# ds2-lab/LambdaFS

Measured on AMD Instinct MI355X. Metric: RS encode+decode GiB/s device-resident; 1/2/4/8 MI355X; %HBM roofline, higher is better.
Workload: dtype u8; 1 GPU; RS(10,4) encode + 1-erasure decode (data shard 0), 1024 KiB cells, 1024 stripes/GPU, device-resident; encodeBulk / decodeBulk via hrs_encode_dev / hrs_decode_dev; stripes_per_gpu=1024, stripes_total=1024, cell_bytes=1048576, k=10, p=4, parallelism=stripe-sharded x1 (RCCL: matrix broadcast + barriers only)

## Files before the change

lambdafs_amd/csrc/hrs_device.hpp:

```cpp
#pragma once
#include <hip/hip_runtime.h>

#include <cstdint>
#include <type_traits>

#include "gf256.hpp"
#include "hrs_crc.hpp"
#include "hrs_internal.hpp"
#include "xor_sched.hpp"

namespace hrs {

typedef uint32_t u32x4 __attribute__((ext_vector_type(4)));

__device__ __forceinline__ uint32_t xor3(uint32_t a, uint32_t b, uint32_t c) {
  return __builtin_amdgcn_bitop3_b32(a, b, c, 0x96);
}

__device__ __forceinline__ uint32_t bsel(uint32_t m, uint32_t x, uint32_t y) {
  return __builtin_amdgcn_bitop3_b32(m, x, y, 0xCA);
}

template <int SH, uint32_t M>
__device__ __forceinline__ void xchg(uint32_t& a, uint32_t& b) {
  const uint32_t na = bsel(M << SH, b << SH, a);
  const uint32_t nb = bsel(M, a >> SH, b);
  a = na;
  b = nb;
}

__device__ __forceinline__ void bitslice(uint32_t (&w)[8]) {
  xchg<1, 0x55555555u>(w[0], w[1]);
  xchg<1, 0x55555555u>(w[2], w[3]);
  xchg<1, 0x55555555u>(w[4], w[5]);
  xchg<1, 0x55555555u>(w[6], w[7]);
  xchg<2, 0x33333333u>(w[0], w[2]);
  xchg<2, 0x33333333u>(w[1], w[3]);
  xchg<2, 0x33333333u>(w[4], w[6]);
  xchg<2, 0x33333333u>(w[5], w[7]);
  xchg<4, 0x0F0F0F0Fu>(w[0], w[4]);
  xchg<4, 0x0F0F0F0Fu>(w[1], w[5]);
  xchg<4, 0x0F0F0F0Fu>(w[2], w[6]);
  xchg<4, 0x0F0F0F0Fu>(w[3], w[7]);
}

__device__ __forceinline__ void xtime(uint32_t (&p)[8]) {
  const uint32_t hi = p[7];
  p[7] = p[6];
  p[6] = p[5];
  p[5] = p[4];
  p[4] = p[3] ^ hi;
  p[3] = p[2] ^ hi;
  p[2] = p[1] ^ hi;
  p[1] = p[0];
  p[0] = hi;
}

__device__ __forceinline__ void load_row(const uint8_t* p, int lane, uint32_t (&w)[8]) {
  const u32x4 x = __builtin_nontemporal_load(reinterpret_cast<const u32x4*>(p + lane * 16));
  const u32x4 y = __builtin_nontemporal_load(reinterpret_cast<const u32x4*>(p + 1024 + lane * 16));
  w[0] = x[0]; w[1] = x[1]; w[2] = x[2]; w[3] = x[3];
  w[4] = y[0]; w[5] = y[1]; w[6] = y[2]; w[7] = y[3];
}

__device__ __forceinline__ void store_row(uint8_t* p, int lane, const uint32_t (&w)[8]) {
  const u32x4 x = {w[0], w[1], w[2], w[3]};
  const u32x4 y = {w[4], w[5], w[6], w[7]};
  __builtin_nontemporal_store(x, reinterpret_cast<u32x4*>(p + lane * 16));
  __builtin_nontemporal_store(y, reinterpret_cast<u32x4*>(p + 1024 + lane * 16));
}

typedef __attribute__((address_space(1))) u32x4 g_u32x4;

__device__ __forceinline__ uint64_t uniform_addr(const void* p) {
  const uint64_t v = reinterpret_cast<uint64_t>(p);
  const uint32_t lo = __builtin_amdgcn_readfirstlane(static_cast<uint32_t>(v));
  const uint32_t hi = __builtin_amdgcn_readfirstlane(static_cast<uint32_t>(v >> 32));
  return (static_cast<uint64_t>(hi) << 32) | lo;
}

__device__ __forceinline__ void load_row_u(const uint8_t* base, uint32_t loff, uint32_t (&w)[8]) {
  const g_u32x4* b = reinterpret_cast<const g_u32x4*>(uniform_addr(base) + loff);
  const u32x4 x = __builtin_nontemporal_load(b);
  const u32x4 y = __builtin_nontemporal_load(b + 64);
  w[0] = x[0]; w[1] = x[1]; w[2] = x[2]; w[3] = x[3];
  w[4] = y[0]; w[5] = y[1]; w[6] = y[2]; w[7] = y[3];
}

__device__ __forceinline__ void store_row_u(uint8_t* base, uint32_t loff, const uint32_t (&w)[8]) {
  g_u32x4* b = reinterpret_cast<g_u32x4*>(uniform_addr(base) + loff);
  const u32x4 x = {w[0], w[1], w[2], w[3]};
  const u32x4 y = {w[4], w[5], w[6], w[7]};
  __builtin_nontemporal_store(x, b);
  __builtin_nontemporal_store(y, b + 64);
}

__device__ __forceinline__ uint32_t wave_id_in_grid() {
  return __builtin_amdgcn_readfirstlane(blockIdx.x * (blockDim.x >> 6) + (threadIdx.x >> 6));
}

struct WaveTasks {
  uint64_t t0, end, jump;
  uint32_t chunk, wpb;

  __device__ __forceinline__ uint64_t at(uint32_t j) const {
    if (chunk == 1) return t0 + j * jump;
    const uint32_t q = j / chunk;
    return t0 + q * jump + static_cast<uint64_t>(j - q * chunk) * wpb;
  }
};

__device__ __forceinline__ WaveTasks wave_tasks(uint64_t ntasks, int order) {
  const uint32_t wpb = blockDim.x >> 6;
  const uint32_t w = __builtin_amdgcn_readfirstlane(threadIdx.x >> 6);
  if (order >= 1) {
    const uint32_t c = static_cast<uint32_t>(order);
    return {static_cast<uint64_t>(blockIdx.x) * c * wpb + w, ntasks, static_cast<uint64_t>(gridDim.x) * c * wpb, c, wpb};
  }
  const uint64_t per = (ntasks + gridDim.x - 1) / gridDim.x;
  const uint64_t lo = per * blockIdx.x;
  return {lo + w, lo + per < ntasks ? lo + per : ntasks, 0, 0xFFFFFFFFu, wpb};
}

template <int K, int P, class MATRIX>
struct StaticPlan {
  uint8_t mask[P][K][8];
  constexpr StaticPlan() : mask{} {
    const MATRIX g;
    for (int o = 0; o < P; ++o)
      for (int r = 0; r < K; ++r)
        for (int q = 0; q < 8; ++q) mask[o][r][q] = gf::row_mask(g.m[o][r], q);
  }
};

template <int K, int P, class MATRIX>
__device__ __forceinline__ void encode_row_acc(int r, const uint32_t (&w)[8], uint32_t (&acc)[P][8],
                                               uint32_t (&pend)[P][8], bool (&has)[P][8]) {
  constexpr StaticPlan<K, P, MATRIX> plan{};
#pragma unroll
  for (int o = 0; o < P; ++o)
#pragma unroll
    for (int q = 0; q < 8; ++q) {
#pragma unroll
      for (int i = 0; i < 8; ++i) {
        if ((plan.mask[o][r][q] >> i) & 1) {
          if (has[o][q]) {
            acc[o][q] = xor3(acc[o][q], pend[o][q], w[i]);
            has[o][q] = false;
          } else {
            pend[o][q] = w[i];
            has[o][q] = true;
          }
        }
      }
    }
}


template <int B, int E, class F>
__device__ __forceinline__ void static_for(F&& f) {
  if constexpr (B < E) {
    f(std::integral_constant<int, B>{});
    static_for<B + 1, E>(f);
  }
}

template <class MATRIX> struct MatrixFamily;
template <int K, int P> struct MatrixFamily<gf::EncodeMatrix<K, P>> { static constexpr int value = 0; };
template <int K, int P> struct MatrixFamily<gf::CauchyMatrix<K, P>> { static constexpr int value = 1; };

template <class S, int GI, int G, int P>
__device__ __forceinline__ void xor_sched_apply(const uint32_t (&x)[G][8], uint32_t (&acc)[P][8]) {
  constexpr int nin = S::kNin[GI];
  constexpr int op0 = S::kOpOff[GI];
  constexpr int nops = S::kOpOff[GI + 1] - op0;
  uint32_t v[S::kMaxVars];
#pragma unroll
  for (int i = 0; i < nin; ++i) v[i] = x[i >> 3][i & 7];
  static_for<0, nops>([&](auto j) __attribute__((always_inline)) {
    constexpr xsched::Op op = S::kOps[op0 + decltype(j)::value];
    if constexpr (op.c == 255)
      v[nin + decltype(j)::value] = v[op.a] ^ v[op.b];
    else
      v[nin + decltype(j)::value] = xor3(v[op.a], v[op.b], v[op.c]);
  });
  static_for<0, 8 * P>([&](auto pl) __attribute__((always_inline)) {
    constexpr int t0 = S::kTermOff[GI][decltype(pl)::value];
    constexpr int t1 = S::kTermOff[GI][decltype(pl)::value + 1];
    uint32_t& a = acc[decltype(pl)::value >> 3][decltype(pl)::value & 7];
    int t = t0;
    if constexpr (GI == 0) {
      if constexpr (t1 == t0) {
        a = 0u;
      } else {
        a = v[S::kTerms[t0]];
        t = t0 + 1;
      }
    }
#pragma unroll
    for (; t + 1 < t1; t += 2) a = xor3(a, v[S::kTerms[t]], v[S::kTerms[t + 1]]);
    if (t < t1) a ^= v[S::kTerms[t]];
  });
}


__device__ __forceinline__ uint32_t zmul(const uint32_t* z, uint32_t c) {
  return z[c & 0xFFu] ^ z[256 + ((c >> 8) & 0xFFu)] ^ z[512 + ((c >> 16) & 0xFFu)] ^ z[768 + (c >> 24)];
}

typedef __attribute__((address_space(3))) const uint32_t lds_u32;

struct SliceTab {
  uint32_t lw_lo;
  uint32_t lw_hi;
};

__device__ __forceinline__ SliceTab slice_tab(int lane, uint32_t rep_mask = kCrcRep - 1) {
  const uint32_t c4 = (static_cast<uint32_t>(lane) & rep_mask) * 4u;
  return SliceTab{c4, c4 | 0x10000u};
}

__device__ __forceinline__ uint32_t lds_at(uint32_t byte_addr) {
  return *reinterpret_cast<lds_u32*>(static_cast<uintptr_t>(byte_addr));
}

__device__ __forceinline__ uint32_t slice4(const SliceTab& t, uint32_t x) {
  const uint32_t a3 = __builtin_amdgcn_perm(x, t.lw_hi, 0x0C020400u);
  const uint32_t a2 = __builtin_amdgcn_perm(x, t.lw_hi, 0x0C020500u);
  const uint32_t a1 = __builtin_amdgcn_perm(x, t.lw_lo, 0x0C0C0600u);
  const uint32_t a0 = __builtin_amdgcn_perm(x, t.lw_lo, 0x0C0C0700u);
  return xor3(lds_at(a3 + 128u), lds_at(a2), lds_at(a1 + 128u)) ^ lds_at(a0);
}

__device__ __forceinline__ uint32_t slice4_xor(const SliceTab& t, uint32_t x, uint32_t y) {
  const uint32_t a3 = __builtin_amdgcn_perm(x, t.lw_hi, 0x0C020400u);
  const uint32_t a2 = __builtin_amdgcn_perm(x, t.lw_hi, 0x0C020500u);
  const uint32_t a1 = __builtin_amdgcn_perm(x, t.lw_lo, 0x0C0C0600u);
  const uint32_t a0 = __builtin_amdgcn_perm(x, t.lw_lo, 0x0C0C0700u);
  return xor3(xor3(lds_at(a3 + 128u), lds_at(a2), lds_at(a1 + 128u)), lds_at(a0), y);
}

__device__ __forceinline__ uint32_t piece_crc(const SliceTab& s, uint32_t w0, uint32_t w1, uint32_t w2, uint32_t w3) {
  uint32_t c = slice4_xor(s, w0, w1);
  c = slice4_xor(s, c, w2);
  c = slice4_xor(s, c, w3);
  return slice4(s, c);
}

__device__ __forceinline__ uint32_t zmul_xor(const uint32_t* z, uint32_t c, uint32_t y) {
  return xor3(xor3(z[c & 0xFFu], z[256 + ((c >> 8) & 0xFFu)], z[512 + ((c >> 16) & 0xFFu)]), z[768 + (c >> 24)], y);
}

template <int M>
__device__ __forceinline__ void rows_piece_crcs(const SliceTab& t, const uint32_t (&x)[M][8], uint32_t (&c0)[M],
                                                uint32_t (&c1)[M]) {
#pragma unroll
  for (int m = 0; m < M; ++m) {
    c0[m] = x[m][0];
    c1[m] = x[m][4];
  }
#pragma unroll
  for (int st = 0; st < 4; ++st) {
#pragma unroll
    for (int m = 0; m < M; ++m) {
      c0[m] = slice4(t, c0[m]);
      c1[m] = slice4(t, c1[m]);
    }
    if (st < 3) {
#pragma unroll
      for (int m = 0; m < M; ++m) {
        c0[m] ^= x[m][st + 1];
        c1[m] ^= x[m][st + 5];
      }
    }
// ... 127 lines not shown
```

lambdafs_amd/csrc/hrs_internal.hpp:

```cpp
#pragma once
#include <cstddef>
#include <cstdint>
#include <hip/hip_runtime.h>

namespace hrs {

constexpr int kMaxIn = 32;
constexpr int kMaxInRuntime = 16;
constexpr int kMaxInRuntimeWide = 8;
inline int runtime_in_chunk(int nout) { return nout <= 5 ? kMaxInRuntime : kMaxInRuntimeWide; }
constexpr int kMaxOut = 8;

constexpr int kWindowBytes = 2048;
constexpr int kBlockThreads = 256;
constexpr int kWavesPerBlock = kBlockThreads / 64;

struct RowArgs {
  const uint8_t* in[kMaxIn];
  uint8_t* out[kMaxOut];
  uint64_t cw[kMaxIn];
  uint64_t in_stride;
  uint64_t out_stride;
  uint64_t len;
  uint64_t nwin;
  uint64_t ntasks;
  int nin;
  int nout;
  int accumulate;
  int order;
};

inline void set_coef(RowArgs& a, int o, int i, uint8_t v) {
  a.cw[i] = (a.cw[i] & ~(0xFFull << (8 * o))) | (static_cast<uint64_t>(v) << (8 * o));
}

enum class KernelKind : int {
  kStaticEncode = 0,
  kBitsliced = 1,
  kBytewise = 2,
};

enum { kStaticRs = 0, kStaticCauchy = 1 };
hipError_t launch_static_encode(int family, int k, int p, const RowArgs& a, hipStream_t s, bool* handled);
hipError_t launch_bitsliced(const RowArgs& a, hipStream_t s);
hipError_t launch_bitsliced_stream(const RowArgs& a, hipStream_t s);
hipError_t launch_bytewise(const RowArgs& a, hipStream_t s);
hipError_t launch_xor(const RowArgs& a, hipStream_t s);
int device_cu_count();

void note_kernel(const char* name);
const char* last_kernel();


constexpr int kBatchMaxIn = 32;
constexpr int kHostBatchSlots = 3;
constexpr int kAsyncSlots = 4;
constexpr int kHostSlots = 8;
struct BatchPlan {
  int nin;
  int nout;
  int loc[kBatchMaxIn];
  uint64_t cw[kBatchMaxIn];
};

struct BatchArgs {
  const uint8_t* base;
  uint8_t* out;
  uint64_t row_stride, stripe_stride, out_row_stride, out_stripe_stride;
  uint64_t len;
  uint64_t col0;
  uint64_t nwin;
  uint64_t ntasks;
  const BatchPlan* plans;
  const int32_t* pat;
  int order;
  int pad_;
};

hipError_t launch_batch_bitsliced(const BatchArgs& a, int max_nout, int max_nin, hipStream_t s);


constexpr int kScrubHead = 4;
constexpr int kScrubPatched = 3;
constexpr uint32_t kScrubNone = 0xFFFFFFFFu;
constexpr int kScrubMaxRows = 255;

struct ScrubArgs {
  const uint8_t* rows[kScrubMaxRows];
  uint64_t stride;
  uint64_t len;
  uint64_t col0;
  uint64_t nwin;
  uint64_t ntasks;
  uint32_t* reports;
  uint64_t report_stride;
  int n, p;
  int order;
  int pad_;
};

hipError_t launch_scrub_init(uint32_t* reports, uint64_t report_stride, int n, uint64_t nstripes, hipStream_t s);
hipError_t launch_scrub(const ScrubArgs& a, hipStream_t s);
hipError_t launch_scrub_bytewise(const ScrubArgs& a, hipStream_t s);
hipError_t launch_heal(const ScrubArgs& a, hipStream_t s);
hipError_t launch_heal_bytewise(const ScrubArgs& a, hipStream_t s);

hipError_t launch_batch_bytewise(const BatchArgs& a, hipStream_t s);

}
```

lambdafs_amd/csrc/hrs_kernels.hip:

```cpp
#include <hip/hip_runtime.h>

#include <cstdlib>
#include <string>

#include "hrs_device.hpp"
#include "hrs_launch.hpp"

namespace hrs {
namespace {


__constant__ gf::Tables d_tables = gf::make_tables();


template <int K, int P, class MATRIX>
__device__ __forceinline__ void encode_static_body(const RowArgs& a) {
  const int lane = threadIdx.x & 63;
  const WaveTasks wt = wave_tasks(a.ntasks, a.order);
  for (uint32_t j = 0; j < 0xFFFFFFFFu; ++j) {
    const uint64_t t = wt.at(j);
    if (t >= wt.end) break;
    const uint64_t stripe = t / a.nwin;
    const uint64_t off = (t - stripe * a.nwin) * kWindowBytes;
    uint32_t acc[P][8];
    uint32_t pend[P][8];
    bool has[P][8];
#pragma unroll
    for (int o = 0; o < P; ++o)
#pragma unroll
      for (int q = 0; q < 8; ++q) {
        acc[o][q] = 0u;
        pend[o][q] = 0u;
        has[o][q] = false;
      }
#pragma unroll
    for (int r = 0; r < K; ++r) {
      uint32_t w[8];
      load_row(a.in[r] + stripe * a.in_stride + off, lane, w);
      bitslice(w);
      encode_row_acc<K, P, MATRIX>(r, w, acc, pend, has);
    }
#pragma unroll
    for (int o = 0; o < P; ++o)
#pragma unroll
      for (int q = 0; q < 8; ++q)
        if (has[o][q]) acc[o][q] ^= pend[o][q];
#pragma unroll
    for (int o = 0; o < P; ++o) {
      bitslice(acc[o]);
      store_row(a.out[o] + stripe * a.out_stride + off, lane, acc[o]);
    }
  }
}

template <int K, int P>
__global__ void __launch_bounds__(kBlockThreads) encode_static_kernel(const RowArgs a) {
  encode_static_body<K, P, gf::EncodeMatrix<K, P>>(a);
}

template <int K, int P>
__global__ void __launch_bounds__(kBlockThreads) encode_cauchy_kernel(const RowArgs a) {
  encode_static_body<K, P, gf::CauchyMatrix<K, P>>(a);
}


template <int NINB>
__global__ void __launch_bounds__(kBlockThreads) xor_kernel(const RowArgs a) {
  const int lane = threadIdx.x & 63;
  const int nin = a.nin;
  const WaveTasks wt = wave_tasks(a.ntasks, a.order);
  for (uint32_t j = 0; j < 0xFFFFFFFFu; ++j) {
    const uint64_t t = wt.at(j);
    if (t >= wt.end) break;
    const uint64_t stripe = t / a.nwin;
    const uint64_t off = (t - stripe * a.nwin) * kWindowBytes;
    const uint64_t in_base = stripe * a.in_stride + off;
    uint32_t rows[NINB][8];
#pragma unroll
    for (int r = 0; r < NINB; ++r)
      if (r < nin) load_row(a.in[r] + in_base, lane, rows[r]);
    uint32_t acc[8];
    if (a.accumulate) {
      load_row(a.out[0] + stripe * a.out_stride + off, lane, acc);
    } else {
#pragma unroll
      for (int q = 0; q < 8; ++q) acc[q] = 0u;
    }
#pragma unroll
    for (int r = 0; r < NINB; r += 2) {
      if (r + 1 < nin) {
#pragma unroll
        for (int q = 0; q < 8; ++q) acc[q] = xor3(acc[q], rows[r][q], rows[r + 1][q]);
      } else if (r < nin) {
#pragma unroll
        for (int q = 0; q < 8; ++q) acc[q] ^= rows[r][q];
      }
    }
    store_row(a.out[0] + stripe * a.out_stride + off, lane, acc);
  }
}


__global__ void __launch_bounds__(kBlockThreads) bytewise_kernel(const RowArgs a) {
  __shared__ uint8_t s_exp[512];
  __shared__ uint8_t s_log[256];
  for (int i = threadIdx.x; i < 512; i += blockDim.x) s_exp[i] = d_tables.exp[i];
  for (int i = threadIdx.x; i < 256; i += blockDim.x) s_log[i] = d_tables.log[i];
  __syncthreads();
  const uint64_t nthreads = static_cast<uint64_t>(gridDim.x) * blockDim.x;
  for (uint64_t idx = static_cast<uint64_t>(blockIdx.x) * blockDim.x + threadIdx.x; idx < a.ntasks;
       idx += nthreads) {
    const uint64_t stripe = idx / a.len;
    const uint64_t col = idx - stripe * a.len;
    uint8_t acc[kMaxOut];
#pragma unroll
    for (int o = 0; o < kMaxOut; ++o)
      acc[o] = (a.accumulate && o < a.nout) ? a.out[o][stripe * a.out_stride + col] : 0;
    for (int r = 0; r < a.nin; ++r) {
      const uint8_t x = a.in[r][stripe * a.in_stride + col];
      if (x == 0) continue;
      const int lx = s_log[x];
#pragma unroll
      for (int o = 0; o < kMaxOut; ++o) {
        const uint8_t c = static_cast<uint8_t>(a.cw[r] >> (8 * o));
        if (o < a.nout && c != 0) acc[o] ^= s_exp[lx + s_log[c]];
      }
    }
#pragma unroll
    for (int o = 0; o < kMaxOut; ++o)
      if (o < a.nout) a.out[o][stripe * a.out_stride + col] = acc[o];
  }
}

template <int K, int P>
hipError_t launch_static(const RowArgs& a, hipStream_t s) {
  auto kern = encode_static_kernel<K, P>;
  note_kernel_t("encode_static_kernel", K, P);
  const unsigned g = stream_grid(a.ntasks);
  hipLaunchKernelGGL(kern, dim3(g), dim3(kBlockThreads), 0, s, with_order(a, kOrderStaticEncode));
  return hipGetLastError();
}

template <int K, int P>
hipError_t launch_cauchy(const RowArgs& a, hipStream_t s) {
  auto kern = encode_cauchy_kernel<K, P>;
  note_kernel_t("encode_cauchy_kernel", K, P);
  const unsigned g = stream_grid(a.ntasks);
  hipLaunchKernelGGL(kern, dim3(g), dim3(kBlockThreads), 0, s, with_order(a, kOrderStaticEncode));
  return hipGetLastError();
}

}

int device_cu_count() { return device_cus(); }

namespace {
thread_local std::string t_last_kernel;
}
void note_kernel(const char* name) { t_last_kernel = name; }
const char* last_kernel() { return t_last_kernel.c_str(); }

hipError_t launch_static_encode(int family, int k, int p, const RowArgs& a, hipStream_t s, bool* handled) {
  *handled = true;
  if (family == kStaticCauchy) {
    if (k == 10 && p == 4) return launch_cauchy<10, 4>(a, s);
    if (k == 6 && p == 3) return launch_cauchy<6, 3>(a, s);
    *handled = false;
    return hipSuccess;
  }
  if (k == 10 && p == 4) return launch_static<10, 4>(a, s);
  if (k == 6 && p == 3) return launch_static<6, 3>(a, s);
  if (k == 3 && p == 2) return launch_static<3, 2>(a, s);
  if (k == 12 && p == 4) return launch_static<12, 4>(a, s);
  *handled = false;
  return hipSuccess;
}

template <int NINB>
hipError_t launch_xor_n(const RowArgs& a, hipStream_t s) {
  auto kern = xor_kernel<NINB>;
  note_kernel_t("xor_kernel", NINB);
  hipLaunchKernelGGL(kern, dim3(stream_grid(a.ntasks)), dim3(kBlockThreads), 0, s, with_order(a, kOrderStaticEncode));
  return hipGetLastError();
}

hipError_t launch_xor(const RowArgs& a, hipStream_t s) {
  if (a.nin <= 4) return launch_xor_n<4>(a, s);
  if (a.nin <= 8) return launch_xor_n<8>(a, s);
  if (a.nin <= 12) return launch_xor_n<12>(a, s);
  if (a.nin <= 16) return launch_xor_n<16>(a, s);
  return hipErrorInvalidValue;
}

hipError_t launch_bytewise(const RowArgs& a, hipStream_t s) {
  const unsigned g = grid_for(bytewise_kernel, kBlockThreads, a.ntasks);
  note_kernel("bytewise_kernel");
  hipLaunchKernelGGL(bytewise_kernel, dim3(g), dim3(kBlockThreads), 0, s, a);
  return hipGetLastError();
}

}
```

lambdafs_amd/csrc/hrs_launch.hpp:

```cpp
#pragma once
#include <hip/hip_runtime.h>

#include <atomic>
#include <cstdint>
#include <cstdlib>
#include <string>
#include <type_traits>

#include "hrs_internal.hpp"

namespace hrs {

inline void kname_arg(std::string& s, int v) { s += std::to_string(v); }
inline void kname_arg(std::string& s, bool v) { s += v ? "true" : "false"; }
inline void kname_arg(std::string& s, const char* v) { s += v; }
template <typename... T>
inline void note_kernel_t(const char* base, T... v) {
  std::string s(base);
  if constexpr (sizeof...(T) > 0) {
    const char* sep = "<";
    ((s += sep, kname_arg(s, v), sep = ", "), ...);
    s += '>';
  }
  note_kernel(s.c_str());
}

template <int Lo, int Hi, class F>
inline hipError_t dispatch_p(int p, F&& f) {
  if constexpr (Lo > Hi) {
    return hipErrorInvalidValue;
  } else {
    constexpr std::integral_constant<int, Lo> P{};
    if (p == Lo) {
      if constexpr (std::is_void_v<decltype(f(P))>) {
        f(P);
        return hipSuccess;
      } else {
        return f(P);
      }
    }
    return dispatch_p<Lo + 1, Hi>(p, f);
  }
}

inline int device_cus() {
  int dev = 0;
  if (hipGetDevice(&dev) != hipSuccess) return 256;
  static std::atomic<int> cus_of[64];
  if (dev < 0 || dev >= 64) return 256;
  int cus = cus_of[dev].load(std::memory_order_relaxed);
  if (cus == 0) {
    if (hipDeviceGetAttribute(&cus, hipDeviceAttributeMultiprocessorCount, dev) != hipSuccess || cus <= 0) cus = 256;
    cus_of[dev].store(cus, std::memory_order_relaxed);
  }
  return cus;
}

inline int task_order(int dflt) {
  const char* e = getenv("HRS_TASK_ORDER");
  if (e && *e) {
    const int c = atoi(e);
    if (c >= 0 && c <= 4096) return c;
  }
  return dflt;
}

constexpr int kOrderStaticEncode = 1;
constexpr int kOrderRuntime = 1;
constexpr int kOrderBatch = 1;
constexpr int kOrderFusedEncode = 1;
constexpr int kOrderDecodeCrc = 1;
constexpr int kOrderCrc = 1;
constexpr int kOrderScrub = 1;

template <class A>
inline A with_order(A a, int dflt) {
  a.order = task_order(dflt);
  return a;
}

inline int blocks_per_cu(int dflt = 2) {
  static int v = [] {
    const char* e = getenv("HRS_BLOCKS_PER_CU");
    int x = e ? atoi(e) : 0;
    return (x >= 1 && x <= 32) ? x : 0;
  }();
  return v ? v : dflt;
}

inline thread_local unsigned t_grid_cap = 0;

struct GridCap {
  unsigned prev;
  explicit GridCap(unsigned cap) : prev(t_grid_cap) { t_grid_cap = cap; }
  ~GridCap() { t_grid_cap = prev; }
};

inline unsigned capped_grid(uint64_t g) {
  if (t_grid_cap && g > t_grid_cap) g = t_grid_cap;
  return static_cast<unsigned>(g == 0 ? 1 : g);
}

inline unsigned stream_grid(uint64_t ntasks, int per_cu = 2) {
  const uint64_t want = static_cast<uint64_t>(blocks_per_cu(per_cu)) * device_cus();
  const uint64_t needed = (ntasks + kWavesPerBlock - 1) / kWavesPerBlock;
  uint64_t g = needed < want ? needed : want;
  return capped_grid(g);
}

template <typename Kernel>
inline unsigned grid_for(Kernel kernel, uint64_t work_items_per_block, uint64_t ntasks) {
  int per_cu = 0;
  if (hipOccupancyMaxActiveBlocksPerMultiprocessor(&per_cu, kernel, kBlockThreads, 0) != hipSuccess ||
      per_cu <= 0)
    per_cu = 2;
  const uint64_t resident = static_cast<uint64_t>(per_cu) * device_cus();
  const uint64_t needed = (ntasks + work_items_per_block - 1) / work_items_per_block;
  uint64_t g = needed < resident ? needed : resident;
  return capped_grid(g);
}

}
```

lambdafs_amd/csrc/hrs_probe.hip:

```cpp
#include <hip/hip_runtime.h>

#include <cstdint>

#include "../../include/hrs_probe.h"
#include "hrs_device.hpp"
#include "hrs_launch.hpp"

namespace hrs {
namespace {

template <bool NT>
__device__ __forceinline__ u32x4 ld16(const u32x4* p) {
  if constexpr (NT) return __builtin_nontemporal_load(p);
  return *p;
}

template <bool NT>
__device__ __forceinline__ void st16(u32x4* p, u32x4 v) {
  if constexpr (NT) __builtin_nontemporal_store(v, p);
  else *p = v;
}

template <int OP, bool NT>
__device__ __forceinline__ void stream_op(const u32x4* __restrict__ src, u32x4* __restrict__ dst, uint64_t i,
                                          u32x4& acc) {
  if constexpr (OP == 0) st16<NT>(&dst[i], ld16<NT>(&src[i]));
  else if constexpr (OP == 1) acc ^= ld16<NT>(&src[i]);
  else st16<NT>(&dst[i], u32x4{static_cast<uint32_t>(i), 0x5A5A5A5Au, ~static_cast<uint32_t>(i), 0u});
}

template <int OP, int D, bool NT>
__device__ __forceinline__ void stream_group(const u32x4* __restrict__ src, u32x4* __restrict__ dst, uint64_t base,
                                             uint64_t step, u32x4& acc) {
  if constexpr (OP == 2) {
#pragma unroll
    for (int j = 0; j < D; ++j) stream_op<2, NT>(src, dst, base + j * step, acc);
  } else {
    u32x4 v[D];
#pragma unroll
    for (int j = 0; j < D; ++j) v[j] = ld16<NT>(&src[base + j * step]);
#pragma unroll
    for (int j = 0; j < D; ++j) {
      if constexpr (OP == 0) st16<NT>(&dst[base + j * step], v[j]);
      else acc ^= v[j];
    }
  }
}

template <int OP, int SCHED, int D, bool NT>
__global__ void __launch_bounds__(1024) stream_kernel(const u32x4* __restrict__ src, u32x4* __restrict__ dst,
                                                       uint64_t n) {
  u32x4 acc = {0u, 0u, 0u, 0u};
  const uint64_t T = static_cast<uint64_t>(gridDim.x) * blockDim.x;
  const uint64_t gid = static_cast<uint64_t>(blockIdx.x) * blockDim.x + threadIdx.x;
  if constexpr (SCHED == HRS_PROBE_WAVE_TASKS) {
    const int lane = threadIdx.x & 63;
    const uint64_t ntasks = n / (64u * D);
    const uint64_t nw = T >> 6;
    for (uint64_t t = gid >> 6; t < ntasks; t += nw) stream_group<OP, D, NT>(src, dst, t * 64u * D + lane, 64u, acc);
    for (uint64_t i = ntasks * 64u * D + gid; i < n; i += T) stream_op<OP, false>(src, dst, i, acc);
  } else if constexpr (SCHED == HRS_PROBE_GRID_STRIDE) {
    uint64_t i = gid;
    for (; i + (D - 1) * T < n; i += D * T) stream_group<OP, D, NT>(src, dst, i, T, acc);
    for (; i < n; i += T) stream_op<OP, false>(src, dst, i, acc);
  } else {
    const uint64_t per = (n + gridDim.x - 1) / gridDim.x;
    const uint64_t lo = per * blockIdx.x;
    const uint64_t hi = lo + per < n ? lo + per : n;
    const uint64_t B = blockDim.x;
    uint64_t i = lo + threadIdx.x;
    for (; i + (D - 1) * B < hi; i += D * B) stream_group<OP, D, NT>(src, dst, i, B, acc);
    for (; i < hi; i += B) stream_op<OP, false>(src, dst, i, acc);
  }
  if constexpr (OP == 1)
    if ((acc[0] ^ acc[1] ^ acc[2] ^ acc[3]) == 0x9E3779B9u && acc[0] == 0x7F4A7C15u) dst[threadIdx.x & 255] = acc;
}

template <int M>
__device__ __forceinline__ u32x4 pace_work(u32x4 x) {
#pragma unroll
  for (int m = 0; m < M; ++m)
#pragma unroll
    for (int q = 0; q < 4; ++q) x[q] = __builtin_amdgcn_alignbit(x[q], x[q], 7) ^ (0x9E3779B9u * (m + 1));
  return x;
}

template <int R, int W, int D, int M>
__global__ void __launch_bounds__(256) rows_kernel(uint8_t* __restrict__ base, uint64_t nstripes, int nrows,
                                                    uint64_t L, int order) {
  const int lane = threadIdx.x & 63;
  const uint64_t nwin = L / 2048u;
  const uint64_t ntasks = nstripes * nwin;
  const WaveTasks wt = wave_tasks(ntasks, order);
  for (uint32_t j = 0; j < 0xFFFFFFFFu; ++j) {
    const uint64_t t = wt.at(j);
    if (t >= wt.end) break;
    const uint64_t s = t / nwin;
    uint8_t* sb = base + s * nrows * L + (t - s * nwin) * 2048u + lane * 16;
    u32x4 v[R][2];
    auto ld = [&](int r) {
      const u32x4* p = reinterpret_cast<const u32x4*>(sb + (nrows - R + r) * L);
      v[r][0] = __builtin_nontemporal_load(p);
      v[r][1] = __builtin_nontemporal_load(p + 64);
    };
#pragma unroll
    for (int r = 0; r < D && r < R; ++r) ld(r);
    u32x4 a = {0u, 0u, 0u, 0u}, b = {0u, 0u, 0u, 0u};
#pragma unroll
    for (int r = 0; r < R; ++r) {
      if (r + D < R) ld(r + D);
      __builtin_amdgcn_sched_barrier(0);
      a ^= pace_work<M>(v[r][0]);
      b ^= pace_work<M>(v[r][1]);
      __builtin_amdgcn_sched_barrier(0);
    }
#pragma unroll
    for (int o = 0; o < W; ++o) {
      u32x4* q = reinterpret_cast<u32x4*>(sb + o * L);
      __builtin_nontemporal_store(a + static_cast<uint32_t>(o), q);
      __builtin_nontemporal_store(b + static_cast<uint32_t>(o), q + 64);
    }
  }
}

template <int OP, int SCHED, int D>
hrs_status launch_stream_d(const void* src, void* dst, uint64_t n, bool nt, unsigned grid, unsigned block,
                           hipStream_t st) {
  auto k = nt ? stream_kernel<OP, SCHED, D, true> : stream_kernel<OP, SCHED, D, false>;
  hipLaunchKernelGGL(k, dim3(grid), dim3(block), 0, st, static_cast<const u32x4*>(src), static_cast<u32x4*>(dst), n);
  return hipGetLastError() == hipSuccess ? HRS_OK : HRS_EDEVICE;
}

template <int OP, int SCHED>
hrs_status launch_stream_s(const void* src, void* dst, uint64_t n, int depth, bool nt, unsigned grid, unsigned block,
                           hipStream_t st) {
  switch (depth) {
    case 1: return launch_stream_d<OP, SCHED, 1>(src, dst, n, nt, grid, block, st);
    case 2: return launch_stream_d<OP, SCHED, 2>(src, dst, n, nt, grid, block, st);
    case 4: return launch_stream_d<OP, SCHED, 4>(src, dst, n, nt, grid, block, st);
    default: return launch_stream_d<OP, SCHED, 8>(src, dst, n, nt, grid, block, st);
  }
}

template <int OP>
hrs_status launch_stream(const void* src, void* dst, size_t bytes, int schedule, int depth, int nt, int block,
                         int bpc, void* stream) {
  const unsigned grid = static_cast<unsigned>(bpc * device_cus());
  const uint64_t n = bytes / 16;
  const hipStream_t st = static_cast<hipStream_t>(stream);
  switch (schedule) {
    case HRS_PROBE_WAVE_TASKS:
      return launch_stream_s<OP, HRS_PROBE_WAVE_TASKS>(src, dst, n, depth, nt != 0, grid, block, st);
    case HRS_PROBE_GRID_STRIDE:
      return launch_stream_s<OP, HRS_PROBE_GRID_STRIDE>(src, dst, n, depth, nt != 0, grid, block, st);
    default:
      return launch_stream_s<OP, HRS_PROBE_BLOCK_RANGE>(src, dst, n, depth, nt != 0, grid, block, st);
  }
}

template <int R, int W, int D, int M>
hrs_status launch_rows_dm(void* base, size_t nstripes, int nrows, size_t L, unsigned grid, hipStream_t st) {
  auto k = rows_kernel<R, W, D, M>;
  hipLaunchKernelGGL(k, dim3(grid), dim3(256), 0, st, static_cast<uint8_t*>(base), static_cast<uint64_t>(nstripes),
                     nrows, static_cast<uint64_t>(L), task_order(kOrderStaticEncode));
  return hipGetLastError() == hipSuccess ? HRS_OK : HRS_EDEVICE;
}

template <int R, int W>
hrs_status launch_rows_rw(void* base, size_t nstripes, int nrows, size_t L, int schedule, unsigned grid,
                          hipStream_t st) {
  switch (schedule) {
    case 0: return launch_rows_dm<R, W, R, 0>(base, nstripes, nrows, L, grid, st);
    case 1: return launch_rows_dm<R, W, 3, 12>(base, nstripes, nrows, L, grid, st);
    case 2: return launch_rows_dm<R, W, 5, 6>(base, nstripes, nrows, L, grid, st);
    default: return launch_rows_dm<R, W, 1, 0>(base, nstripes, nrows, L, grid, st);
  }
}

bool stream_args_ok(int schedule, int depth, int block, int bpc) {
  return schedule >= HRS_PROBE_WAVE_TASKS && schedule <= HRS_PROBE_BLOCK_RANGE &&
         (depth == 1 || depth == 2 || depth == 4 || depth == 8) && (block == 256 || block == 512 || block == 1024) &&
         bpc >= 1 && bpc * block <= 8192;
}

}
}

extern "C" hrs_status hrs_probe_stream(int op, const void* src, void* dst, size_t bytes, int schedule, int depth,
                                       int nontemporal, int block_threads, int blocks_per_cu, void* stream) {
  if (op < HRS_PROBE_COPY || op > HRS_PROBE_WRITE || !hrs::stream_args_ok(schedule, depth, block_threads, blocks_per_cu))
    return HRS_EINVAL;
  const bool need_src = op != HRS_PROBE_WRITE;
  if (bytes && ((need_src && !src) || !dst)) return HRS_EINVAL;
  if ((reinterpret_cast<uintptr_t>(src) | reinterpret_cast<uintptr_t>(dst) | bytes) & 15u) return HRS_EALIGN;
  if (bytes == 0) return HRS_OK;
  switch (op) {
    case HRS_PROBE_COPY:
      return hrs::launch_stream<0>(src, dst, bytes, schedule, depth, nontemporal, block_threads, blocks_per_cu, stream);
    case HRS_PROBE_READ:
      return hrs::launch_stream<1>(src, dst, bytes, schedule, depth, nontemporal, block_threads, blocks_per_cu, stream);
    default:
      return hrs::launch_stream<2>(nullptr, dst, bytes, schedule, depth, nontemporal, block_threads, blocks_per_cu,
                                   stream);
  }
}

extern "C" hrs_status hrs_probe_rows(void* base, size_t nstripes, int nrows, size_t cell_bytes, int nread,
                                     int nwrite, int schedule, int blocks_per_cu, void* stream) {
  if (blocks_per_cu < 1 || blocks_per_cu > 32 || nrows < 1 || nread < 1 || nwrite < 0 || nread + nwrite > nrows ||
      schedule < 0 || schedule > 3)
    return HRS_EINVAL;
  if (nstripes && !base) return HRS_EINVAL;
  if ((reinterpret_cast<uintptr_t>(base) & 15u) || (cell_bytes % 2048u)) return HRS_EALIGN;
  if (nstripes == 0 || cell_bytes == 0) return HRS_OK;
  const unsigned grid = static_cast<unsigned>(blocks_per_cu * hrs::device_cus());
  const hipStream_t st = static_cast<hipStream_t>(stream);
  switch (nread * 100 + nwrite) {
    case 1004: return hrs::launch_rows_rw<10, 4>(base, nstripes, nrows, cell_bytes, schedule, grid, st);
    case 1003: return hrs::launch_rows_rw<10, 3>(base, nstripes, nrows, cell_bytes, schedule, grid, st);
    case 1002: return hrs::launch_rows_rw<10, 2>(base, nstripes, nrows, cell_bytes, schedule, grid, st);
    case 1001: return hrs::launch_rows_rw<10, 1>(base, nstripes, nrows, cell_bytes, schedule, grid, st);
    case 1000: return hrs::launch_rows_rw<10, 0>(base, nstripes, nrows, cell_bytes, schedule, grid, st);
    case 603: return hrs::launch_rows_rw<6, 3>(base, nstripes, nrows, cell_bytes, schedule, grid, st);
    case 1204: return hrs::launch_rows_rw<12, 4>(base, nstripes, nrows, cell_bytes, schedule, grid, st);
    case 1202: return hrs::launch_rows_rw<12, 2>(base, nstripes, nrows, cell_bytes, schedule, grid, st);
    case 302: return hrs::launch_rows_rw<3, 2>(base, nstripes, nrows, cell_bytes, schedule, grid, st);
    default: return HRS_EINVAL;
  }
}
```

lambdafs_amd/csrc/hrs_runtime.hip:

```cpp
#include <hip/hip_runtime.h>

#include <cstdlib>

#include "hrs_device.hpp"
#include "hrs_launch.hpp"

namespace hrs {
namespace {

template <int NOUT, int NINB>
__global__ void __launch_bounds__(kBlockThreads) bitsliced_kernel(const RowArgs a) {
  const int lane = threadIdx.x & 63;
  const WaveTasks wt = wave_tasks(a.ntasks, a.order);
  for (uint32_t j = 0; j < 0xFFFFFFFFu; ++j) {
    const uint64_t t = wt.at(j);
    if (t >= wt.end) break;
    int nin = a.nin;
    asm volatile("" : "+s"(nin));
    const uint64_t stripe = t / a.nwin;
    const uint64_t off = (t - stripe * a.nwin) * kWindowBytes;
    const uint64_t in_base = stripe * a.in_stride + off;
    uint32_t rows[NINB][8];
#pragma unroll
    for (int r = 0; r < NINB; ++r)
      if (r < nin) load_row(a.in[r] + in_base, lane, rows[r]);
    uint32_t acc[NOUT][8];
    if (a.accumulate) {
#pragma unroll
      for (int o = 0; o < NOUT; ++o) {
        load_row(a.out[o] + stripe * a.out_stride + off, lane, acc[o]);
        bitslice(acc[o]);
      }
    } else {
#pragma unroll
      for (int o = 0; o < NOUT; ++o)
#pragma unroll
        for (int q = 0; q < 8; ++q) acc[o][q] = 0u;
    }
#pragma unroll
    for (int r = 0; r < NINB; ++r) {
      if (r < nin) accumulate_row<NOUT, NINB>(acc, rows[r], a.cw[r]);
    }
#pragma unroll
    for (int o = 0; o < NOUT; ++o) {
      bitslice(acc[o]);
      store_row(a.out[o] + stripe * a.out_stride + off, lane, acc[o]);
    }
  }
}

template <int NOUT, int NINB>
__device__ __forceinline__ void load_task(const RowArgs& a, uint64_t t, int nin, int lane,
                                          uint32_t (&rows)[NINB][8]) {
  const uint64_t stripe = t / a.nwin;
  const uint64_t off = (t - stripe * a.nwin) * kWindowBytes;
  const uint64_t in_base = stripe * a.in_stride + off;
#pragma unroll
  for (int r = 0; r < NINB; ++r)
    if (r < nin) load_row(a.in[r] + in_base, lane, rows[r]);
}

template <int NOUT, int NINB>
__device__ __forceinline__ void apply_task(const RowArgs& a, uint64_t t, int nin, int lane,
                                           uint32_t (&rows)[NINB][8]) {
  const uint64_t stripe = t / a.nwin;
  const uint64_t off = (t - stripe * a.nwin) * kWindowBytes;
  uint32_t acc[NOUT][8];
  if (a.accumulate) {
#pragma unroll
    for (int o = 0; o < NOUT; ++o) {
      load_row(a.out[o] + stripe * a.out_stride + off, lane, acc[o]);
      bitslice(acc[o]);
    }
  } else {
#pragma unroll
    for (int o = 0; o < NOUT; ++o)
#pragma unroll
      for (int q = 0; q < 8; ++q) acc[o][q] = 0u;
  }
#pragma unroll
  for (int r = 0; r < NINB; ++r) {
    if (r < nin) accumulate_row<NOUT, NINB>(acc, rows[r], a.cw[r]);
  }
#pragma unroll
  for (int o = 0; o < NOUT; ++o) {
    bitslice(acc[o]);
    store_row(a.out[o] + stripe * a.out_stride + off, lane, acc[o]);
  }
}

template <int NOUT, int NINB>
__global__ void __launch_bounds__(kBlockThreads) bitsliced_pipe_kernel(const RowArgs a) {
  static_assert(!BitLoop<NOUT, NINB>::kRolled, "pipelined kernel takes the unrolled shapes only");
  const int lane = threadIdx.x & 63;
  int nin = a.nin;
  asm volatile("" : "+s"(nin));
  const WaveTasks wt = wave_tasks(a.ntasks, a.order);
  uint32_t j = 0;
  uint64_t t = wt.at(0);
  if (t >= wt.end) return;
  uint32_t ra[NINB][8], rb[NINB][8];
  load_task<NOUT, NINB>(a, t, nin, lane, ra);
  for (;;) {
    const uint64_t t1 = wt.at(++j);
    if (t1 < wt.end) load_task<NOUT, NINB>(a, t1, nin, lane, rb);
    apply_task<NOUT, NINB>(a, t, nin, lane, ra);
    if (t1 >= wt.end) break;
    const uint64_t t2 = wt.at(++j);
    if (t2 < wt.end) load_task<NOUT, NINB>(a, t2, nin, lane, ra);
    apply_task<NOUT, NINB>(a, t1, nin, lane, rb);
    if (t2 >= wt.end) break;
    t = t2;
  }
}

template <int NOUT, int D>
__device__ __forceinline__ void load_group(const RowArgs& a, int r0, int nin, uint64_t in_base, int lane,
                                           uint32_t (&rows)[D][8]) {
#pragma unroll
  for (int j = 0; j < D; ++j)
    if (r0 + j < nin) load_row(a.in[r0 + j] + in_base, lane, rows[j]);
}

template <int NOUT, int D>
__device__ __forceinline__ void acc_group(const RowArgs& a, int r0, int nin, uint32_t (&acc)[NOUT][8],
                                          uint32_t (&rows)[D][8]) {
  constexpr int kNinb = NOUT >= 4 ? 16 : 8;
#pragma unroll
  for (int j = 0; j < D; ++j)
    if (r0 + j < nin) accumulate_row<NOUT, kNinb>(acc, rows[j], a.cw[r0 + j]);
}

template <int NOUT, int D>
__global__ void __launch_bounds__(kBlockThreads) bitsliced_stream_kernel(const RowArgs a) {
  const int lane = threadIdx.x & 63;
  const WaveTasks wt = wave_tasks(a.ntasks, a.order);
  for (uint32_t j = 0; j < 0xFFFFFFFFu; ++j) {
    const uint64_t t = wt.at(j);
    if (t >= wt.end) break;
    int nin = a.nin;
    asm volatile("" : "+s"(nin));
    const uint64_t stripe = t / a.nwin;
    const uint64_t off = (t - stripe * a.nwin) * kWindowBytes;
    const uint64_t in_base = stripe * a.in_stride + off;
    uint32_t acc[NOUT][8];
    if (a.accumulate) {
#pragma unroll
      for (int o = 0; o < NOUT; ++o) {
        load_row(a.out[o] + stripe * a.out_stride + off, lane, acc[o]);
        bitslice(acc[o]);
      }
    } else {
#pragma unroll
      for (int o = 0; o < NOUT; ++o)
#pragma unroll
        for (int q = 0; q < 8; ++q) acc[o][q] = 0u;
    }
    uint32_t ra[D][8], rb[D][8];
    load_group<NOUT, D>(a, 0, nin, in_base, lane, ra);
#pragma unroll 1
    for (int r0 = 0; r0 < nin; r0 += 2 * D) {
      if (r0 + D < nin) load_group<NOUT, D>(a, r0 + D, nin, in_base, lane, rb);
      acc_group<NOUT, D>(a, r0, nin, acc, ra);
      if (r0 + D >= nin) break;
      if (r0 + 2 * D < nin) load_group<NOUT, D>(a, r0 + 2 * D, nin, in_base, lane, ra);
      acc_group<NOUT, D>(a, r0 + D, nin, acc, rb);
    }
#pragma unroll
    for (int o = 0; o < NOUT; ++o) {
      bitslice(acc[o]);
      store_row(a.out[o] + stripe * a.out_stride + off, lane, acc[o]);
    }
  }
}

constexpr int kStreamGroup = 4;

template <int NOUT, int NINB>
constexpr bool kPipeFits = !BitLoop<NOUT, NINB>::kRolled && 16 * NINB + 8 * NOUT <= 232;

bool use_pipe() {
  static bool v = [] {
    const char* e = getenv("HRS_PIPE");
    return !(e && e[0] == '0');
  }();
  return v;
}

template <int NOUT, int NINB>
hipError_t launch_bits_n(const RowArgs& a, hipStream_t s) {
  auto kern = bitsliced_kernel<NOUT, NINB>;
  const char* name = "bitsliced_kernel";
  if constexpr (kPipeFits<NOUT, NINB>)
    if (use_pipe()) {
      kern = bitsliced_pipe_kernel<NOUT, NINB>;
      name = "bitsliced_pipe_kernel";
    }
  note_kernel_t(name, NOUT, NINB);
  const int per_cu = BitLoop<NOUT, NINB>::kRolled ? 3 : 2;
  hipLaunchKernelGGL(kern, dim3(stream_grid(a.ntasks, per_cu)), dim3(kBlockThreads), 0, s, with_order(a, kOrderRuntime));
  return hipGetLastError();
}

template <int NOUT>
hipError_t launch_bits(const RowArgs& a, hipStream_t s) {
  if (a.nin <= 4) return launch_bits_n<NOUT, 4>(a, s);
  if (a.nin <= 8) return launch_bits_n<NOUT, 8>(a, s);
  if constexpr (NOUT < 6) {
    if (a.nin <= 12) return launch_bits_n<NOUT, 12>(a, s);
    if (a.nin <= 16) return launch_bits_n<NOUT, 16>(a, s);
  }
  return hipErrorInvalidValue;
}

template <int NOUT>
hipError_t launch_stream_n(const RowArgs& a, hipStream_t s) {
  auto kern = bitsliced_stream_kernel<NOUT, kStreamGroup>;
  note_kernel_t("bitsliced_stream_kernel", NOUT, kStreamGroup);
  const int per_cu = NOUT >= 4 ? 3 : 2;
  hipLaunchKernelGGL(kern, dim3(stream_grid(a.ntasks, per_cu)), dim3(kBlockThreads), 0, s, with_order(a, kOrderRuntime));
  return hipGetLastError();
}

}

hipError_t launch_bitsliced_stream(const RowArgs& a, hipStream_t s) {
  if (a.nin < 1 || a.nin > kMaxIn) return hipErrorInvalidValue;
  switch (a.nout) {
    case 1: return launch_stream_n<1>(a, s);
    case 2: return launch_stream_n<2>(a, s);
    case 3: return launch_stream_n<3>(a, s);
    case 4: return launch_stream_n<4>(a, s);
    case 5: return launch_stream_n<5>(a, s);
    case 6: return launch_stream_n<6>(a, s);
    case 7: return launch_stream_n<7>(a, s);
    case 8: return launch_stream_n<8>(a, s);
    default: return hipErrorInvalidValue;
  }
}

hipError_t launch_bitsliced(const RowArgs& a, hipStream_t s) {
  switch (a.nout) {
    case 1: return launch_bits<1>(a, s);
    case 2: return launch_bits<2>(a, s);
    case 3: return launch_bits<3>(a, s);
    case 4: return launch_bits<4>(a, s);
    case 5: return launch_bits<5>(a, s);
    case 6: return launch_bits<6>(a, s);
    case 7: return launch_bits<7>(a, s);
    case 8: return launch_bits<8>(a, s);
    default: return hipErrorInvalidValue;
  }
}

}
```

Measured before the change: 4138 GiB/s.

## Split each task's two 1 KiB pieces across distant halves of a window group

Adds a window-to-offset mapping in which each wave task loads its two 1 KiB pieces from positions separated by a configurable stride (default 32 KiB) rather than adjacent 1 KiB pieces. Neighbouring tasks then touch contiguous 1 KiB runs, which changes the DRAM/channel access pattern of the encode, decode and probe kernels. The stride is plumbed through RowArgs and can be overridden with an environment variable. It keeps per-byte correctness because bitslicing pairs pieces consistently across inputs and outputs, but adds index arithmetic and may hurt locality per wave.

```diff
diff --git a/lambdafs_amd/csrc/hrs_device.hpp b/lambdafs_amd/csrc/hrs_device.hpp
--- a/lambdafs_amd/csrc/hrs_device.hpp
+++ b/lambdafs_amd/csrc/hrs_device.hpp
@@ -7,6 +7,7 @@
 #include "gf256.hpp"
 #include "hrs_crc.hpp"
 #include "hrs_internal.hpp"
+#include "hrs_window_map.hpp"
 #include "xor_sched.hpp"
 
 namespace hrs {
@@ -56,18 +57,18 @@
   p[0] = hi;
 }
 
-__device__ __forceinline__ void load_row(const uint8_t* p, int lane, uint32_t (&w)[8]) {
+__device__ __forceinline__ void load_row(const uint8_t* p, int lane, uint32_t (&w)[8], uint32_t half = 1024) {
   const u32x4 x = __builtin_nontemporal_load(reinterpret_cast<const u32x4*>(p + lane * 16));
-  const u32x4 y = __builtin_nontemporal_load(reinterpret_cast<const u32x4*>(p + 1024 + lane * 16));
+  const u32x4 y = __builtin_nontemporal_load(reinterpret_cast<const u32x4*>(p + half + lane * 16));
   w[0] = x[0]; w[1] = x[1]; w[2] = x[2]; w[3] = x[3];
   w[4] = y[0]; w[5] = y[1]; w[6] = y[2]; w[7] = y[3];
 }
 
-__device__ __forceinline__ void store_row(uint8_t* p, int lane, const uint32_t (&w)[8]) {
+__device__ __forceinline__ void store_row(uint8_t* p, int lane, const uint32_t (&w)[8], uint32_t half = 1024) {
   const u32x4 x = {w[0], w[1], w[2], w[3]};
   const u32x4 y = {w[4], w[5], w[6], w[7]};
   __builtin_nontemporal_store(x, reinterpret_cast<u32x4*>(p + lane * 16));
-  __builtin_nontemporal_store(y, reinterpret_cast<u32x4*>(p + 1024 + lane * 16));
+  __builtin_nontemporal_store(y, reinterpret_cast<u32x4*>(p + half + lane * 16));
 }
 
 typedef __attribute__((address_space(1))) u32x4 g_u32x4;
@@ -120,6 +121,17 @@
   const uint64_t per = (ntasks + gridDim.x - 1) / gridDim.x;
   const uint64_t lo = per * blockIdx.x;
   return {lo + w, lo + per < ntasks ? lo + per : ntasks, 0, 0xFFFFFFFFu, wpb};
+}
+
+struct TaskPos {
+  uint64_t stripe, off;
+  uint32_t half;
+};
+
+__device__ __forceinline__ TaskPos task_pos(const RowArgs& a, uint64_t t) {
+  const uint64_t stripe = t / a.nwin;
+  const WindowPos wp = window_pos(t - stripe * a.nwin, a.nwin, a.split);
+  return {stripe, wp.off, wp.half};
 }
 
 template <int K, int P, class MATRIX>
diff --git a/lambdafs_amd/csrc/hrs_internal.hpp b/lambdafs_amd/csrc/hrs_internal.hpp
--- a/lambdafs_amd/csrc/hrs_internal.hpp
+++ b/lambdafs_amd/csrc/hrs_internal.hpp
@@ -28,6 +28,7 @@
   int nout;
   int accumulate;
   int order;
+  int split;
 };
 
 inline void set_coef(RowArgs& a, int o, int i, uint8_t v) {
diff --git a/lambdafs_amd/csrc/hrs_kernels.hip b/lambdafs_amd/csrc/hrs_kernels.hip
--- a/lambdafs_amd/csrc/hrs_kernels.hip
+++ b/lambdafs_amd/csrc/hrs_kernels.hip
@@ -20,8 +20,8 @@
   for (uint32_t j = 0; j < 0xFFFFFFFFu; ++j) {
     const uint64_t t = wt.at(j);
     if (t >= wt.end) break;
-    const uint64_t stripe = t / a.nwin;
-    const uint64_t off = (t - stripe * a.nwin) * kWindowBytes;
+    const TaskPos tp = task_pos(a, t);
+    const uint64_t stripe = tp.stripe, off = tp.off;
     uint32_t acc[P][8];
     uint32_t pend[P][8];
     bool has[P][8];
@@ -36,7 +36,7 @@
 #pragma unroll
     for (int r = 0; r < K; ++r) {
       uint32_t w[8];
-      load_row(a.in[r] + stripe * a.in_stride + off, lane, w);
+      load_row(a.in[r] + stripe * a.in_stride + off, lane, w, tp.half);
       bitslice(w);
       encode_row_acc<K, P, MATRIX>(r, w, acc, pend, has);
     }
@@ -48,7 +48,7 @@
 #pragma unroll
     for (int o = 0; o < P; ++o) {
       bitslice(acc[o]);
-      store_row(a.out[o] + stripe * a.out_stride + off, lane, acc[o]);
+      store_row(a.out[o] + stripe * a.out_stride + off, lane, acc[o], tp.half);
     }
   }
 }
@@ -137,7 +137,8 @@
   auto kern = encode_static_kernel<K, P>;
   note_kernel_t("encode_static_kernel", K, P);
   const unsigned g = stream_grid(a.ntasks);
-  hipLaunchKernelGGL(kern, dim3(g), dim3(kBlockThreads), 0, s, with_order(a, kOrderStaticEncode));
+  hipLaunchKernelGGL(kern, dim3(g), dim3(kBlockThreads), 0, s,
+                     with_split(with_order(a, kOrderStaticEncode), kSplitStaticEncode));
   return hipGetLastError();
 }
 
@@ -146,7 +147,8 @@
   auto kern = encode_cauchy_kernel<K, P>;
   note_kernel_t("encode_cauchy_kernel", K, P);
   const unsigned g = stream_grid(a.ntasks);
-  hipLaunchKernelGGL(kern, dim3(g), dim3(kBlockThreads), 0, s, with_order(a, kOrderStaticEncode));
+  hipLaunchKernelGGL(kern, dim3(g), dim3(kBlockThreads), 0, s,
+                     with_split(with_order(a, kOrderStaticEncode), kSplitStaticEncode));
   return hipGetLastError();
 }
 
diff --git a/lambdafs_amd/csrc/hrs_launch.hpp b/lambdafs_amd/csrc/hrs_launch.hpp
--- a/lambdafs_amd/csrc/hrs_launch.hpp
+++ b/lambdafs_amd/csrc/hrs_launch.hpp
@@ -8,6 +8,7 @@
 #include <type_traits>
 
 #include "hrs_internal.hpp"
+#include "hrs_window_map.hpp"
 
 namespace hrs {
 
@@ -79,6 +80,24 @@
   return a;
 }
 
+inline int window_split(int dflt_bytes) {
+  const char* e = getenv("HRS_WINDOW_SPLIT");
+  if (e && *e) {
+    const int s = split_of_bytes(atoll(e));
+    if (s >= 0) return s;
+  }
+  return split_of_bytes(dflt_bytes);
+}
+
+constexpr int kSplitStaticEncode = 32768;
+constexpr int kSplitRuntime = 32768;
+
+template <class A>
+inline A with_split(A a, int dflt_bytes) {
+  a.split = window_split(dflt_bytes);
+  return a;
+}
+
 inline int blocks_per_cu(int dflt = 2) {
   static int v = [] {
     const char* e = getenv("HRS_BLOCKS_PER_CU");
diff --git a/lambdafs_amd/csrc/hrs_probe.hip b/lambdafs_amd/csrc/hrs_probe.hip
--- a/lambdafs_amd/csrc/hrs_probe.hip
+++ b/lambdafs_amd/csrc/hrs_probe.hip
@@ -87,7 +87,7 @@
 
 template <int R, int W, int D, int M>
 __global__ void __launch_bounds__(256) rows_kernel(uint8_t* __restrict__ base, uint64_t nstripes, int nrows,
-                                                    uint64_t L, int order) {
+                                                    uint64_t L, int order, int split) {
   const int lane = threadIdx.x & 63;
   const uint64_t nwin = L / 2048u;
   const uint64_t ntasks = nstripes * nwin;
@@ -96,12 +96,14 @@
     const uint64_t t = wt.at(j);
     if (t >= wt.end) break;
     const uint64_t s = t / nwin;
-    uint8_t* sb = base + s * nrows * L + (t - s * nwin) * 2048u + lane * 16;
+    const WindowPos wp = window_pos(t - s * nwin, nwin, split);
+    const uint32_t half16 = wp.half / 16;
+    uint8_t* sb = base + s * nrows * L + wp.off + lane * 16;
     u32x4 v[R][2];
     auto ld = [&](int r) {
       const u32x4* p = reinterpret_cast<const u32x4*>(sb + (nrows - R + r) * L);
       v[r][0] = __builtin_nontemporal_load(p);
-      v[r][1] = __builtin_nontemporal_load(p + 64);
+      v[r][1] = __builtin_nontemporal_load(p + half16);
     };
 #pragma unroll
     for (int r = 0; r < D && r < R; ++r) ld(r);
@@ -118,7 +120,7 @@
     for (int o = 0; o < W; ++o) {
       u32x4* q = reinterpret_cast<u32x4*>(sb + o * L);
       __builtin_nontemporal_store(a + static_cast<uint32_t>(o), q);
-      __builtin_nontemporal_store(b + static_cast<uint32_t>(o), q + 64);
+      __builtin_nontemporal_store(b + static_cast<uint32_t>(o), q + half16);
     }
   }
 }
@@ -158,11 +160,16 @@
   }
 }
 
+constexpr bool static_encode_mix(int r, int w) {
+  return (r == 10 && w == 4) || (r == 6 && w == 3) || (r == 12 && w == 4) || (r == 3 && w == 2);
+}
+
 template <int R, int W, int D, int M>
 hrs_status launch_rows_dm(void* base, size_t nstripes, int nrows, size_t L, unsigned grid, hipStream_t st) {
   auto k = rows_kernel<R, W, D, M>;
   hipLaunchKernelGGL(k, dim3(grid), dim3(256), 0, st, static_cast<uint8_t*>(base), static_cast<uint64_t>(nstripes),
-                     nrows, static_cast<uint64_t>(L), task_order(kOrderStaticEncode));
+                     nrows, static_cast<uint64_t>(L), task_order(kOrderStaticEncode),
+                     window_split(static_encode_mix(R, W) ? kSplitStaticEncode : kSplitRuntime));
   return hipGetLastError() == hipSuccess ? HRS_OK : HRS_EDEVICE;
 }
 
diff --git a/lambdafs_amd/csrc/hrs_runtime.hip b/lambdafs_amd/csrc/hrs_runtime.hip
--- a/lambdafs_amd/csrc/hrs_runtime.hip
+++ b/lambdafs_amd/csrc/hrs_runtime.hip
@@ -17,18 +17,18 @@
     if (t >= wt.end) break;
     int nin = a.nin;
     asm volatile("" : "+s"(nin));
-    const uint64_t stripe = t / a.nwin;
-    const uint64_t off = (t - stripe * a.nwin) * kWindowBytes;
+    const TaskPos tp = task_pos(a, t);
+    const uint64_t stripe = tp.stripe, off = tp.off;
     const uint64_t in_base = stripe * a.in_stride + off;
     uint32_t rows[NINB][8];
 #pragma unroll
     for (int r = 0; r < NINB; ++r)
-      if (r < nin) load_row(a.in[r] + in_base, lane, rows[r]);
+      if (r < nin) load_row(a.in[r] + in_base, lane, rows[r], tp.half);
     uint32_t acc[NOUT][8];
     if (a.accumulate) {
 #pragma unroll
       for (int o = 0; o < NOUT; ++o) {
-        load_row(a.out[o] + stripe * a.out_stride + off, lane, acc[o]);
+        load_row(a.out[o] + stripe * a.out_stride + off, lane, acc[o], tp.half);
         bitslice(acc[o]);
       }
     } else {
@@ -44,7 +44,7 @@
 #pragma unroll
     for (int o = 0; o < NOUT; ++o) {
       bitslice(acc[o]);
-      store_row(a.out[o] + stripe * a.out_stride + off, lane, acc[o]);
+      store_row(a.out[o] + stripe * a.out_stride + off, lane, acc[o], tp.half);
     }
   }
 }
@@ -52,24 +52,24 @@
 template <int NOUT, int NINB>
 __device__ __forceinline__ void load_task(const RowArgs& a, uint64_t t, int nin, int lane,
                                           uint32_t (&rows)[NINB][8]) {
-  const uint64_t stripe = t / a.nwin;
-  const uint64_t off = (t - stripe * a.nwin) * kWindowBytes;
+  const TaskPos tp = task_pos(a, t);
+  const uint64_t stripe = tp.stripe, off = tp.off;
   const uint64_t in_base = stripe * a.in_stride + off;
 #pragma unroll
   for (int r = 0; r < NINB; ++r)
-    if (r < nin) load_row(a.in[r] + in_base, lane, rows[r]);
+    if (r < nin) load_row(a.in[r] + in_base, lane, rows[r], tp.half);
 }
 
 template <int NOUT, int NINB>
 __device__ __forceinline__ void apply_task(const RowArgs& a, uint64_t t, int nin, int lane,
                                            uint32_t (&rows)[NINB][8]) {
-  const uint64_t stripe = t / a.nwin;
-  const uint64_t off = (t - stripe * a.nwin) * kWindowBytes;
+  const TaskPos tp = task_pos(a, t);
+  const uint64_t stripe = tp.stripe, off = tp.off;
   uint32_t acc[NOUT][8];
   if (a.accumulate) {
 #pragma unroll
     for (int o = 0; o < NOUT; ++o) {
-      load_row(a.out[o] + stripe * a.out_stride + off, lane, acc[o]);
+      load_row(a.out[o] + stripe * a.out_stride + off, lane, acc[o], tp.half);
       bitslice(acc[o]);
     }
   } else {
@@ -85,7 +85,7 @@
 #pragma unroll
   for (int o = 0; o < NOUT; ++o) {
     bitslice(acc[o]);
-    store_row(a.out[o] + stripe * a.out_stride + off, lane, acc[o]);
+    store_row(a.out[o] + stripe * a.out_stride + off, lane, acc[o], tp.half);
   }
 }
 
@@ -115,11 +115,11 @@
 }
 
 template <int NOUT, int D>
-__device__ __forceinline__ void load_group(const RowArgs& a, int r0, int nin, uint64_t in_base, int lane,
-                                           uint32_t (&rows)[D][8]) {
+__device__ __forceinline__ void load_group(const RowArgs& a, int r0, int nin, uint64_t in_base, uint32_t half,
+                                           int lane, uint32_t (&rows)[D][8]) {
 #pragma unroll
   for (int j = 0; j < D; ++j)
-    if (r0 + j < nin) load_row(a.in[r0 + j] + in_base, lane, rows[j]);
+    if (r0 + j < nin) load_row(a.in[r0 + j] + in_base, lane, rows[j], half);
 }
 
 template <int NOUT, int D>
@@ -140,14 +140,14 @@
     if (t >= wt.end) break;
     int nin = a.nin;
     asm volatile("" : "+s"(nin));
-    const uint64_t stripe = t / a.nwin;
-    const uint64_t off = (t - stripe * a.nwin) * kWindowBytes;
+    const TaskPos tp = task_pos(a, t);
+    const uint64_t stripe = tp.stripe, off = tp.off;
     const uint64_t in_base = stripe * a.in_stride + off;
     uint32_t acc[NOUT][8];
     if (a.accumulate) {
 #pragma unroll
       for (int o = 0; o < NOUT; ++o) {
-        load_row(a.out[o] + stripe * a.out_stride + off, lane, acc[o]);
+        load_row(a.out[o] + stripe * a.out_stride + off, lane, acc[o], tp.half);
         bitslice(acc[o]);
       }
     } else {
@@ -157,19 +157,19 @@
         for (int q = 0; q < 8; ++q) acc[o][q] = 0u;
     }
     uint32_t ra[D][8], rb[D][8];
-    load_group<NOUT, D>(a, 0, nin, in_base, lane, ra);
+    load_group<NOUT, D>(a, 0, nin, in_base, tp.half, lane, ra);
 #pragma unroll 1
     for (int r0 = 0; r0 < nin; r0 += 2 * D) {
-      if (r0 + D < nin) load_group<NOUT, D>(a, r0 + D, nin, in_base, lane, rb);
+      if (r0 + D < nin) load_group<NOUT, D>(a, r0 + D, nin, in_base, tp.half, lane, rb);
       acc_group<NOUT, D>(a, r0, nin, acc, ra);
       if (r0 + D >= nin) break;
-      if (r0 + 2 * D < nin) load_group<NOUT, D>(a, r0 + 2 * D, nin, in_base, lane, ra);
+      if (r0 + 2 * D < nin) load_group<NOUT, D>(a, r0 + 2 * D, nin, in_base, tp.half, lane, ra);
       acc_group<NOUT, D>(a, r0 + D, nin, acc, rb);
     }
 #pragma unroll
     for (int o = 0; o < NOUT; ++o) {
       bitslice(acc[o]);
-      store_row(a.out[o] + stripe * a.out_stride + off, lane, acc[o]);
+      store_row(a.out[o] + stripe * a.out_stride + off, lane, acc[o], tp.half);
     }
   }
 }
@@ -198,7 +198,8 @@
     }
   note_kernel_t(name, NOUT, NINB);
   const int per_cu = BitLoop<NOUT, NINB>::kRolled ? 3 : 2;
-  hipLaunchKernelGGL(kern, dim3(stream_grid(a.ntasks, per_cu)), dim3(kBlockThreads), 0, s, with_order(a, kOrderRuntime));
+  hipLaunchKernelGGL(kern, dim3(stream_grid(a.ntasks, per_cu)), dim3(kBlockThreads), 0, s,
+                     with_split(with_order(a, kOrderRuntime), kSplitRuntime));
   return hipGetLastError();
 }
 
@@ -218,7 +219,8 @@
   auto kern = bitsliced_stream_kernel<NOUT, kStreamGroup>;
   note_kernel_t("bitsliced_stream_kernel", NOUT, kStreamGroup);
   const int per_cu = NOUT >= 4 ? 3 : 2;
-  hipLaunchKernelGGL(kern, dim3(stream_grid(a.ntasks, per_cu)), dim3(kBlockThreads), 0, s, with_order(a, kOrderRuntime));
+  hipLaunchKernelGGL(kern, dim3(stream_grid(a.ntasks, per_cu)), dim3(kBlockThreads), 0, s,
+                     with_split(with_order(a, kOrderRuntime), kSplitRuntime));
   return hipGetLastError();
 }
 
diff --git a/lambdafs_amd/csrc/hrs_window_map.hpp b/lambdafs_amd/csrc/hrs_window_map.hpp
--- /dev/null
+++ b/lambdafs_amd/csrc/hrs_window_map.hpp
@@ -0,0 +1,36 @@
+#pragma once
+#include <cstdint>
+
+#if defined(__HIPCC__) || defined(__CUDACC__)
+#define HRS_HD __host__ __device__ __forceinline__
+#else
+#define HRS_HD inline
+#endif
+
+namespace hrs {
+
+constexpr uint32_t kPieceBytes = 1024;
+constexpr uint32_t kSplitMinBytes = 1024;
+constexpr uint32_t kSplitMaxBytes = 1 << 20;
+
+struct WindowPos {
+  uint64_t off;
+  uint32_t half;
+};
+
+HRS_HD WindowPos window_pos(uint64_t w, uint64_t nwin, int split) {
+  const uint64_t strided = (nwin >> split) << split;
+  if (w >= strided) return {w * (2 * kPieceBytes), kPieceBytes};
+  const uint64_t g = w >> split;
+  const uint64_t c = w - (g << split);
+  return {(g << (split + 11)) + c * kPieceBytes, kPieceBytes << split};
+}
+
+HRS_HD int split_of_bytes(int64_t h) {
+  if (h < kSplitMinBytes || h > kSplitMaxBytes || (h & (h - 1)) != 0) return -1;
+  int s = 0;
+  while ((int64_t{kPieceBytes} << s) < h) ++s;
+  return s;
+}
+
+}
```

New measurement: 4671 GiB/s, median of 6. 12.9% higher.
